# YuanxunLu/LiveSpeechPortraits

Measured on NVIDIA H100. Metric: 512x512 frames/sec (Feature2Face_G large / May.yaml), higher is better.
Workload: dtype fp16 hi+lo split operands (3 wgmma MMAs per K step), fp32 accumulate

## Files before the change

### livespeechportraits_b200/csrc/conv_wgmma.cuh

```cuda
#pragma once
#include <cuda_bf16.h>
#include <cuda_fp16.h>
#include "ptx.cuh"

namespace lspg {

constexpr int kTileM = 128;
constexpr int kChunk = 64;
constexpr int kATile = kTileM * 128;
constexpr int kMaxTaps = 9;
constexpr int kThreads = 384;
constexpr int kSmemBudget = 227 * 1024;

struct FastDiv {
  uint32_t mul, shr, d;
};
inline FastDiv make_fast_div(uint32_t d) {
  FastDiv f;
  f.d = d; f.mul = 0; f.shr = 0;
  if (d > 1) {
    uint32_t l = 0;
    while ((1u << l) < d) ++l;
    const uint64_t pw = 31 + l;
    f.mul = static_cast<uint32_t>(((1ull << pw) + d - 1) / d);
// ... 257 lines not shown
}

template <int CL>
__device__ __forceinline__ void release_stage(uint64_t* bar) {
  if constexpr (CL == 1) ptx::mbar_arrive(bar);
  else {
#pragma unroll
    for (int c = 0; c < CL; ++c) ptx::mbar_arrive_cluster(bar, static_cast<uint32_t>(c));
  }
}

template <int BN, int NL, bool TAIL>
__global__ void __launch_bounds__(kThreads, 1) conv_umma_kernel(const __grid_constant__ ConvParams p) {
  using Cfg = ConvCfg<BN, NL, TAIL>;
  const int t0 = static_cast<int>(blockIdx.x), tstep = static_cast<int>(gridDim.x);
  extern __shared__ uint8_t smem_raw[];
  uint8_t* smem = reinterpret_cast<uint8_t*>((reinterpret_cast<uintptr_t>(smem_raw) + 1023) & ~uintptr_t(1023));
  uint8_t* aux = smem + Cfg::kStages * Cfg::kStage;
  uint64_t* full_bar = reinterpret_cast<uint64_t*>(aux);
  uint64_t* empty_bar = full_bar + Cfg::kStages;
  float* tail_stg = reinterpret_cast<float*>(aux + kBarBytes);

  const int warp = __shfl_sync(0xffffffffu, static_cast<int>(threadIdx.x >> 5), 0);
  const int lane = threadIdx.x & 31;
  if (threadIdx.x == 0) { trace_stamp(p, 0); trace_time(p, false); }

  if (warp == 0 && lane == 0) {
    for (int i = 0; i < 4; ++i) ptx::prefetch_tmap(&p.a[i]);
    ptx::prefetch_tmap(&p.w);
    for (int i = 0; i < Cfg::kStages; ++i) {
      ptx::mbar_init(&full_bar[i], 1);
      ptx::mbar_init(&empty_bar[i], 2);
    }
    ptx::fence_mbar_init();
  }
  __syncthreads();
  ptx::pdl_launch_dependents();
  if (threadIdx.x == 0) trace_stamp(p, 1);

  int kb_per_tap = 0;
  for (int s = 0; s < p.n_src; ++s) kb_per_tap += p.chunks[s];
  const int num_kb = p.n_taps * kb_per_tap;

  if (warp == 0) {
    int pre = 0;
    if (t0 < p.total_tiles) {
      const TileCoord tc = decode_tile(p, t0);
      const int kb0 = tc.split * p.split_len;
      const int kb1 = (kb0 + p.split_len < num_kb) ? kb0 + p.split_len : num_kb;
      pre = (kb1 - kb0 < Cfg::kStages) ? kb1 - kb0 : Cfg::kStages;
      if (ptx::elect_one()) {
        for (int i = 0; i < pre; ++i) {
          uint8_t* st = smem + i * Cfg::kStage;
          ptx::mbar_expect_tx(&full_bar[i], Cfg::kStage);
#pragma unroll
          for (int l = 0; l < NL; ++l)
            ptx::tma_load_3d(&p.w, &full_bar[i], st + NL * kATile + l * Cfg::kBTile, (kb0 + i) * kChunk, tc.nt * BN,
                             l * p.n_phases + tc.z);
        }
      }
      __syncwarp();
    }
    ptx::pdl_wait();
    int stage = 0;
    uint32_t phase = 0;
    int issued = 0;
    int lt = 0;
    for (int t = t0; t < p.total_tiles; t += tstep, ++lt) {
      const TileCoord tc = decode_tile(p, t);
      const int kb0 = tc.split * p.split_len;
      const int kb1 = (kb0 + p.split_len < num_kb) ? kb0 + p.split_len : num_kb;
      if (lane == 0) trace_tile(p, lt, 6);
      for (int kb = kb0; kb < kb1; ++kb, ++issued) {
        const int tap = kb / kb_per_tap;
        const int rem = kb - tap * kb_per_tap;
        const int s = (rem < p.chunks[0]) ? 0 : 1;
        const int c = s ? rem - p.chunks[0] : rem;
        const int amap = p.tap_map[tc.z][tap];
        const int xx = tc.x0 + p.tap_dx[tc.z][tap];
        const int yy = tc.y0 + p.tap_dy[tc.z][tap];
        const bool early = issued < pre;
        if (!early) ptx::mbar_wait(&empty_bar[stage], phase ^ 1);
        if (ptx::elect_one()) {
          uint8_t* st = smem + stage * Cfg::kStage;
          if (!early) ptx::mbar_expect_tx(&full_bar[stage], Cfg::kStage);
#pragma unroll
          for (int l = 0; l < NL; ++l) {
            ptx::tma_load_5d(&p.a[amap + s], &full_bar[stage], st + l * kATile, c * kChunk, xx, yy, tc.n0, l);
            if (!early)
              ptx::tma_load_3d(&p.w, &full_bar[stage], st + NL * kATile + l * Cfg::kBTile, kb * kChunk, tc.nt * BN,
                               l * p.n_phases + tc.z);
          }
        }
        __syncwarp();
        if (++stage == Cfg::kStages) { stage = 0; phase ^= 1; }
      }
      if (lane == 0) trace_tile(p, lt, 7);
    }
  } else if (warp >= 4) {
    ptx::pdl_wait();
    const int cw = (warp >> 2) - 1;
    const bool wg_leader = (threadIdx.x & 127) == 0;
    int stage = 0;
    uint32_t phase = 0;
    int lt = 0;
    for (int t = t0; t < p.total_tiles; t += tstep, ++lt) {
      const TileCoord tc = decode_tile(p, t);
      const int kb0 = tc.split * p.split_len;
      const int kb1 = (kb0 + p.split_len < num_kb) ? kb0 + p.split_len : num_kb;
      if (threadIdx.x == 128) trace_tile(p, lt, 0);
      float acc[BN / 2];
#pragma unroll
      for (int i = 0; i < BN / 2; ++i) acc[i] = 0.0f;
      int prev = -1;
      for (int kb = kb0; kb < kb1; ++kb) {
        ptx::mbar_wait(&full_bar[stage], phase);
        if (threadIdx.x == 128 && kb == kb0) trace_tile(p, lt, 1);
        ptx::wgmma_fence();
        const uint32_t a0 = ptx::smem_u32(smem + stage * Cfg::kStage) + cw * 64 * 128;
        const uint32_t b0 = ptx::smem_u32(smem + stage * Cfg::kStage) + NL * kATile;
        const uint64_t a_hi = ptx::gmma_desc_sw128(a0);
        const uint64_t b_hi = ptx::gmma_desc_sw128(b0);
#pragma unroll
        for (int k = 0; k < kChunk / 16; ++k) {
          const uint32_t accum = (kb > kb0 || k > 0) ? 1u : 0u;
          ptx::wgmma_m64k16<BN, NL == 2>(acc, a_hi + 2 * k, b_hi + 2 * k, accum);
          if constexpr (NL == 2) {
            const uint64_t a_lo = ptx::gmma_desc_sw128(a0 + kATile);
            const uint64_t b_lo = ptx::gmma_desc_sw128(b0 + Cfg::kBTile);
            ptx::wgmma_m64k16<BN, true>(acc, a_hi + 2 * k, b_lo + 2 * k, 1u);
            ptx::wgmma_m64k16<BN, true>(acc, a_lo + 2 * k, b_hi + 2 * k, 1u);
          }
        }
        ptx::wgmma_commit();
        ptx::wgmma_wait<1>();
        if (prev >= 0 && wg_leader) release_stage<1>(&empty_bar[prev]);
        prev = stage;
        if (++stage == Cfg::kStages) { stage = 0; phase ^= 1; }
      }
      ptx::wgmma_wait<0>();
      if (prev >= 0 && wg_leader) release_stage<1>(&empty_bar[prev]);
      if (threadIdx.x == 128) trace_tile(p, lt, 2);
      epilogue_regs<BN, NL, TAIL>(p, acc, tc, t, 64 * cw, tail_stg + cw * 64 * kTailStride, 1 + cw);
      if (threadIdx.x == 128) trace_tile(p, lt, 3);
    }
  }
  if (threadIdx.x == 0) trace_time(p, true);
}


constexpr int kPatchSlot = 23 * 1024;
constexpr int kPatchStride = 23 * 1024;

constexpr int kProducerRegs = 40;
constexpr int kConsumerRegs = 232;
static_assert(128 * kProducerRegs + 256 * kConsumerRegs <= 65536, "register file of one SM");

template <int BN, int NL, bool TAIL>
struct PatchCfg {
  using Aux = AuxCfg<TAIL, 2 * kTileM>;
  static constexpr int kBTile = BN * 128;
  static constexpr int kTPS = TAIL ? 9 : (BN >= 128 ? (NL == 1 ? 2 : 1) : (NL == 1 ? 3 : 2));
  static constexpr int kAStage = NL * kPatchStride;
  static constexpr int kBStage = NL * kTPS * kBTile;
  static constexpr int kAStages = 2;
  static constexpr int kAvail = kSmemBudget - 1024 - Aux::kBytes - kAStages * kAStage;
  static constexpr int kBStagesRaw = kAvail / kBStage;
  static constexpr int kBStages = kBStagesRaw > 12 ? 12 : kBStagesRaw;
  static constexpr int kSmemBytes = 1024 + kAStages * kAStage + kBStages * kBStage + Aux::kBytes;
  static_assert(kBStages >= 2, "B ring needs at least two stages");
  static_assert(BN == 16 || BN == 64 || BN == 128, "instantiated N tiles");
};

template <int BN, int NL, bool TAIL, int CL>
__global__ void __launch_bounds__(kThreads, 1) conv_patch_kernel(const __grid_constant__ ConvParams p) {
  using Cfg = PatchCfg<BN, NL, TAIL>;
  const int t0 = static_cast<int>(blockIdx.x), tstep = static_cast<int>(gridDim.x);
  extern __shared__ uint8_t smem_raw[];
  uint8_t* smem = reinterpret_cast<uint8_t*>((reinterpret_cast<uintptr_t>(smem_raw) + 1023) & ~uintptr_t(1023));
  uint8_t* a_ring = smem;
  uint8_t* b_ring = a_ring + Cfg::kAStages * Cfg::kAStage;
  uint8_t* aux = b_ring + Cfg::kBStages * Cfg::kBStage;
  uint64_t* afull_bar = reinterpret_cast<uint64_t*>(aux);
  uint64_t* aempty_bar = afull_bar + Cfg::kAStages;
  uint64_t* bfull_bar = aempty_bar + Cfg::kAStages;
  uint64_t* bempty_bar = bfull_bar + Cfg::kBStages;
  uint64_t* turn_bar = bempty_bar + Cfg::kBStages;
  float* tail_stg = reinterpret_cast<float*>(aux + kBarBytes);

  const int warp = __shfl_sync(0xffffffffu, static_cast<int>(threadIdx.x >> 5), 0);
  const int lane = threadIdx.x & 31;
  if (threadIdx.x == 0) { trace_stamp(p, 0); trace_time(p, false); }

  if (warp == 0 && lane == 0) {
    for (int i = 0; i < 4; ++i) ptx::prefetch_tmap(&p.a[i]);
    ptx::prefetch_tmap(&p.w);
    for (int i = 0; i < Cfg::kAStages; ++i) { ptx::mbar_init(&afull_bar[i], 1); ptx::mbar_init(&aempty_bar[i], 1); }
    for (int i = 0; i < Cfg::kBStages; ++i) { ptx::mbar_init(&bfull_bar[i], 1); ptx::mbar_init(&bempty_bar[i], CL); }
    for (int i = 0; i < 2; ++i) ptx::mbar_init(&turn_bar[i], 1);
    ptx::fence_mbar_init();
  }
  __syncthreads();
  if (CL > 1) ptx::cluster_sync();
  const uint32_t crank = (CL > 1) ? ptx::cluster_ctarank() : 0u;
  constexpr uint16_t kMask = static_cast<uint16_t>((1u << CL) - 1u);
  ptx::pdl_launch_dependents();
  if (threadIdx.x == 0) trace_stamp(p, 1);

  int kb_per_tap = 0;
  for (int s = 0; s < p.n_src; ++s) kb_per_tap += p.chunks[s];
  const int patch_bytes = p.patch_w * p.patch_h * 128;
  const int n_groups = (p.n_taps + Cfg::kTPS - 1) / Cfg::kTPS;

  if (warp < 4) {
    ptx::setmaxnreg_dec<kProducerRegs>();
    if (warp == 0) {
      ptx::pdl_wait();
      int ia = 0, ib = 0;
      uint32_t pha = 0, phb = 0;
      int a_tile = t0, a_ci = -1;
      auto issue_a = [&]() {
        if (a_tile >= p.total_tiles) return;
        const TileCoord tc = decode_tile(p, a_tile);
        const int ci0 = tc.split * p.split_len;
        const int ci1 = (ci0 + p.split_len < kb_per_tap) ? ci0 + p.split_len : kb_per_tap;
        if (a_ci < 0) a_ci = ci0;
        const int s = (a_ci < p.chunks[0]) ? 0 : 1;
        const int c = (s == 0) ? a_ci : a_ci - p.chunks[0];
        ptx::mbar_wait(&aempty_bar[ia], pha ^ 1);
        if (ptx::elect_one()) {
          ptx::mbar_expect_tx(&afull_bar[ia], NL * patch_bytes);
#pragma unroll
          for (int l = 0; l < NL; ++l)
            ptx::tma_load_5d(&p.a[s], &afull_bar[ia], a_ring + ia * Cfg::kAStage + l * kPatchStride, c * kChunk,
                             tc.x0 + p.patch_dx0[tc.z], tc.y0 + p.patch_dy0[tc.z], tc.n0, l);
        }
        __syncwarp();
        if (++ia == Cfg::kAStages) { ia = 0; pha ^= 1; }
        if (++a_ci == ci1) { a_ci = -1; a_tile += tstep; }
      };
      issue_a();
      const int a_after_group = (n_groups > 1) ? 1 : 0;
      int lt = 0;
      for (int t = t0; t < p.total_tiles; t += tstep, ++lt) {
        const TileCoord tc = decode_tile(p, t);
        const int ci0 = tc.split * p.split_len;
        const int ci1 = (ci0 + p.split_len < kb_per_tap) ? ci0 + p.split_len : kb_per_tap;
        if (lane == 0) trace_tile(p, lt, 6);
        for (int ci = ci0; ci < ci1; ++ci) {
          for (int g = 0; g < n_groups; ++g) {
            ptx::mbar_wait(&bempty_bar[ib], phb ^ 1);
            if (ptx::elect_one()) {
              uint8_t* st = b_ring + ib * Cfg::kBStage;
              if constexpr (CL == 1 && NL == 1) {
                ptx::mbar_expect_tx(&bfull_bar[ib], Cfg::kBStage);
                ptx::tma_load_4d(&p.w, &bfull_bar[ib], st, ci * kChunk, tc.nt * BN, g * Cfg::kTPS, tc.z);
              } else {
                const int tap0 = g * Cfg::kTPS;
                const int ntap = (tap0 + Cfg::kTPS < p.n_taps) ? Cfg::kTPS : p.n_taps - tap0;
                ptx::mbar_expect_tx(&bfull_bar[ib], NL * ntap * Cfg::kBTile);
                constexpr int kRows = BN / CL;
                for (int ti = 0; ti < ntap; ++ti)
#pragma unroll
                  for (int l = 0; l < NL; ++l) {
                    uint8_t* dst = st + (ti * NL + l) * Cfg::kBTile + crank * kRows * 128;
                    if constexpr (CL == 1)
                      ptx::tma_load_4d(&p.w, &bfull_bar[ib], dst, ci * kChunk, tc.nt * BN, tap0 + ti, l * p.n_phases + tc.z);
                    else
                      ptx::tma_load_4d_mc(&p.w, &bfull_bar[ib], dst, ci * kChunk, tc.nt * BN + crank * kRows, tap0 + ti,
                                          l * p.n_phases + tc.z, kMask);
                  }
              }
            }
            __syncwarp();
            if (++ib == Cfg::kBStages) { ib = 0; phb ^= 1; }
            if (g == a_after_group) issue_a();
          }
        }
        if (lane == 0) trace_tile(p, lt, 7);
      }
    }
  } else {
    ptx::setmaxnreg_inc<kConsumerRegs>();
    ptx::pdl_wait();
    const int wg = (warp >> 2) - 1;
    const bool wg_leader = (threadIdx.x & 127) == 0;
    int ia = 0, ib = 0;
    uint32_t pha = 0, phb = 0;
    const uint32_t sbo = static_cast<uint32_t>(p.patch_w) * 128u;
    const uint32_t row_off = static_cast<uint32_t>(8 * p.patch_w) * 128u;
    const bool boff = p.desc_base_offset != 0;
    float* stg = tail_stg + wg * kTileM * kTailStride;
    int lt = 0;
    for (int t = t0; t < p.total_tiles; t += tstep, ++lt) {
      const TileCoord tc = decode_tile(p, t);
      const int ci0 = tc.split * p.split_len;
      const int ci1 = (ci0 + p.split_len < kb_per_tap) ? ci0 + p.split_len : kb_per_tap;
      if ((lt & 1) != wg) {
        ia += ci1 - ci0;
        pha ^= static_cast<uint32_t>(ia / Cfg::kAStages) & 1u;
        ia %= Cfg::kAStages;
        ib += (ci1 - ci0) * n_groups;
        phb ^= static_cast<uint32_t>(ib / Cfg::kBStages) & 1u;
        ib %= Cfg::kBStages;
        continue;
      }
      if (lt > 0) ptx::mbar_wait(&turn_bar[wg ^ 1], static_cast<uint32_t>((lt - 1) >> 1) & 1u);
      if (wg_leader) trace_tile(p, lt, 0);
      float acc[2][BN / 2];
#pragma unroll
      for (int h = 0; h < 2; ++h)
#pragma unroll
        for (int i = 0; i < BN / 2; ++i) acc[h][i] = 0.0f;
      int prev_b = -1, prev_a = -1;
      for (int ci = ci0; ci < ci1; ++ci) {
        ptx::mbar_wait(&afull_bar[ia], pha);
        const uint32_t a0 = ptx::smem_u32(a_ring + ia * Cfg::kAStage);
        for (int g = 0; g < n_groups; ++g) {
          ptx::mbar_wait(&bfull_bar[ib], phb);
          if (wg_leader && ci == ci0 && g == 0) trace_tile(p, lt, 1);
          ptx::wgmma_fence();
          const int tap0 = g * Cfg::kTPS;
          const uint32_t b0 = ptx::smem_u32(b_ring + ib * Cfg::kBStage);
#pragma unroll
          for (int i = 0; i < Cfg::kTPS; ++i) {
            const int tap = tap0 + i;
            if (i == 0 || tap < p.n_taps) {
              const uint32_t a_hi_addr = a0 + static_cast<uint32_t>(p.tap_row[tc.z][tap]) * 128u;
              const uint32_t b_hi_addr = b0 + static_cast<uint32_t>(i) * (NL * Cfg::kBTile);
              const uint64_t b_hi = ptx::gmma_desc_sw128(b_hi_addr);
              const uint64_t b_lo = ptx::gmma_desc_sw128(b_hi_addr + Cfg::kBTile);
#pragma unroll
              for (int k = 0; k < kChunk / 16; ++k) {
                const uint32_t accum = (ci > ci0 || tap > 0 || k > 0) ? 1u : 0u;
#pragma unroll
                for (int h = 0; h < 2; ++h) {
                  const uint64_t a_hi = ptx::gmma_desc_sw128(a_hi_addr + h * row_off, sbo, boff);
                  ptx::wgmma_m64k16<BN, NL == 2>(acc[h], a_hi + 2 * k, b_hi + 2 * k, accum);
                  if constexpr (NL == 2) {
                    const uint64_t a_lo = ptx::gmma_desc_sw128(a_hi_addr + h * row_off + kPatchStride, sbo, boff);
                    ptx::wgmma_m64k16<BN, true>(acc[h], a_hi + 2 * k, b_lo + 2 * k, 1u);
                    ptx::wgmma_m64k16<BN, true>(acc[h], a_lo + 2 * k, b_hi + 2 * k, 1u);
                  }
                }
              }
            }
          }
          ptx::wgmma_commit();
          if (ci == ci1 - 1 && g == n_groups - 1 && wg_leader) ptx::mbar_arrive(&turn_bar[wg]);
          ptx::wgmma_wait<1>();
          if (wg_leader) {
            if (prev_b >= 0) release_stage<CL>(&bempty_bar[prev_b]);
            if (prev_a >= 0) ptx::mbar_arrive(&aempty_bar[prev_a]);
          }
          prev_b = ib;
          prev_a = (g == n_groups - 1) ? ia : -1;
          if (++ib == Cfg::kBStages) { ib = 0; phb ^= 1; }
        }
        if (++ia == Cfg::kAStages) { ia = 0; pha ^= 1; }
      }
      ptx::wgmma_wait<0>();
      if (wg_leader) {
        if (prev_b >= 0) release_stage<CL>(&bempty_bar[prev_b]);
        if (prev_a >= 0) ptx::mbar_arrive(&aempty_bar[prev_a]);
      }
      if (wg_leader) trace_tile(p, lt, 2);
#pragma unroll
      for (int h = 0; h < 2; ++h)
        epilogue_regs<BN, NL, TAIL>(p, acc[h], tc, t, 64 * h, stg + 64 * h * kTailStride, 1 + wg);
      if (wg_leader) trace_tile(p, lt, 3);
    }
  }
  if (CL > 1) ptx::cluster_sync();
  if (threadIdx.x == 0) trace_time(p, true);
}

struct ReduceParams {
  const float* partial;
  const float* scale;
  const float* shift;
  const __nv_bfloat16* res;
  long long res_limb_stride;
  __nv_bfloat16* out;
  long long out_limb_stride;
  int32_t n_split, tiles_per_split, m_tiles, n_tiles, n_phases;
  int32_t tiles_x, tiles_y, tw_log2, th_log2, bn;
  int32_t batch, hs, ws, up, channels, relu, has_res, nl;
};

__global__ void __launch_bounds__(128) splitk_reduce_kernel(const ReduceParams p) {
  ptx::pdl_wait();
  ptx::pdl_launch_dependents();
  const int groups = p.bn >> 2;
  const long long total = static_cast<long long>(p.tiles_per_split) * kTileM * groups;
  for (long long e = blockIdx.x * static_cast<long long>(blockDim.x) + threadIdx.x; e < total;
       e += static_cast<long long>(gridDim.x) * blockDim.x) {
    const int g = static_cast<int>(e % groups);
    const long long r0 = e / groups;
    const int row = static_cast<int>(r0 % kTileM);
    const int tile = static_cast<int>(r0 / kTileM);
    const int mt = tile % p.m_tiles;
    const int r1 = tile / p.m_tiles;
    const int nt = r1 % p.n_tiles;
    const int z = r1 / p.n_tiles;
    const int tx = mt % p.tiles_x;
    const int r2 = mt / p.tiles_x;
    const int ty = r2 % p.tiles_y;
    const int tn = r2 / p.tiles_y;
    const int tw = row & ((1 << p.tw_log2) - 1);
    const int th = (row >> p.tw_log2) & ((1 << p.th_log2) - 1);
    const int nb = row >> (p.tw_log2 + p.th_log2);
    const int n = (tn << (7 - p.tw_log2 - p.th_log2)) + nb;
    const int y = (ty << p.th_log2) + th, x = (tx << p.tw_log2) + tw;
    if (n >= p.batch || y >= p.hs || x >= p.ws) continue;
    float acc[4] = {0.f, 0.f, 0.f, 0.f};
    const size_t split_stride = static_cast<size_t>(p.tiles_per_split) * kTileM * p.bn;
    const float* src0 = p.partial + (static_cast<size_t>(tile) * kTileM + row) * p.bn + g * 4;
    int s = 0;
    for (; s + 16 <= p.n_split; s += 16) {
      float4 v[16];
#pragma unroll
      for (int u = 0; u < 16; ++u) v[u] = *reinterpret_cast<const float4*>(src0 + (s + u) * split_stride);
#pragma unroll
      for (int u = 0; u < 16; ++u) {
        acc[0] += v[u].x; acc[1] += v[u].y; acc[2] += v[u].z; acc[3] += v[u].w;
      }
    }
    for (; s + 4 <= p.n_split; s += 4) {
      float4 v[4];
#pragma unroll
      for (int u = 0; u < 4; ++u) v[u] = *reinterpret_cast<const float4*>(src0 + (s + u) * split_stride);
#pragma unroll
      for (int u = 0; u < 4; ++u) { acc[0] += v[u].x; acc[1] += v[u].y; acc[2] += v[u].z; acc[3] += v[u].w; }
    }
    for (; s < p.n_split; ++s) {
      const float4 a = *reinterpret_cast<const float4*>(src0 + s * split_stride);
      acc[0] += a.x; acc[1] += a.y; acc[2] += a.z; acc[3] += a.w;
    }
    const int ch = nt * p.bn + g * 4;
    const int oh = p.up ? 2 * p.hs : p.hs, ow = p.up ? 2 * p.ws : p.ws;
    const int oy = p.up ? 2 * y + (z >> 1) : y, ox = p.up ? 2 * x + (z & 1) : x;
    const size_t off = ((static_cast<size_t>(n) * oh + oy) * ow + ox) * p.channels + ch;
    const float4 sc = *reinterpret_cast<const float4*>(p.scale + ch), sh = *reinterpret_cast<const float4*>(p.shift + ch);
    float yv[4] = {fmaf(acc[0], sc.x, sh.x), fmaf(acc[1], sc.y, sh.y), fmaf(acc[2], sc.z, sh.z), fmaf(acc[3], sc.w, sh.w)};
    if (p.has_res) {
      for (int l = 0; l < p.nl; ++l) {
        const uint2 r = *reinterpret_cast<const uint2*>(p.res + l * p.res_limb_stride + off);
        if (p.nl == 2) {
          yv[0] += unpack_lo<true>(r.x); yv[1] += unpack_hi<true>(r.x); yv[2] += unpack_lo<true>(r.y); yv[3] += unpack_hi<true>(r.y);
        } else {
          yv[0] += bf16_lo(r.x); yv[1] += bf16_hi(r.x); yv[2] += bf16_lo(r.y); yv[3] += bf16_hi(r.y);
        }
      }
    }
    if (p.relu) {
#pragma unroll
      for (int i = 0; i < 4; ++i) yv[i] = fmaxf(yv[i], 0.f);
    }
    if (p.nl == 2) {
      uint2 o, lo;
      o.x = pack2<true>(yv[0], yv[1]); o.y = pack2<true>(yv[2], yv[3]);
      lo.x = pack2<true>(yv[0] - unpack_lo<true>(o.x), yv[1] - unpack_hi<true>(o.x));
      lo.y = pack2<true>(yv[2] - unpack_lo<true>(o.y), yv[3] - unpack_hi<true>(o.y));
      *reinterpret_cast<uint2*>(p.out + off) = o;
      *reinterpret_cast<uint2*>(p.out + p.out_limb_stride + off) = lo;
    } else {
      uint2 o;
      o.x = pack_bf16x2(yv[0], yv[1]); o.y = pack_bf16x2(yv[2], yv[3]);
      *reinterpret_cast<uint2*>(p.out + off) = o;
    }
  }
}

}
```

### livespeechportraits_b200/csrc/lspg.cu

```cuda
#include <cuda.h>
#include <cuda_runtime.h>

#include <algorithm>
#include <cmath>
#include <cstdarg>
#include <cstdio>
#include <cstdlib>
#include <cstring>
#include <functional>
#include <map>
#include <memory>
#include <string>
#include <tuple>
#include <utility>
#include <vector>

#include "../../include/lspg.h"
#include "aux_kernels.cuh"
#include "raster.cuh"
#include "conv_wgmma.cuh"

namespace {

using namespace lspg;
// ... 592 lines not shown
    p.n_tiles = L.cout_pad / pl.bn;
    p.n_phases = L.n_phases;
    p.tiles_per_split = g.tiles_per_split;
    p.fd_tps = make_fast_div(g.tiles_per_split);
    p.fd_m_tiles = make_fast_div(p.tiles_x * p.tiles_y * p.tiles_n);
    p.fd_n_tiles = make_fast_div(p.n_tiles);
    p.fd_tiles_x = make_fast_div(p.tiles_x);
    p.fd_tiles_y = make_fast_div(p.tiles_y);
    p.n_split = g.n_split; p.split_len = g.split_len;
    p.total_tiles = g.tiles_per_split * g.n_split;
    p.partial = reinterpret_cast<float*>(ws_scratch);
    pl.split = g.n_split > 1;
    p.n_taps = L.n_taps; p.n_src = L.n_src;
    p.chunks[0] = L.cin[0] / 64; p.chunks[1] = L.n_src == 2 ? L.cin[1] / 64 : 0;
    p.relu = L.relu; p.has_res = L.res >= 0 ? 1 : 0;
    p.batch = B; p.hs = Hs; p.ws = Ws;
    const bool f16 = NL > 1;
    p.scale = f16 ? L.d_scale_par : L.d_scale; p.shift = L.d_shift; p.out_f32 = nullptr;
    memcpy(p.tap_map, L.tap_map, sizeof(p.tap_map));
    memcpy(p.tap_dx, L.tap_dx, sizeof(p.tap_dx));
    memcpy(p.tap_dy, L.tap_dy, sizeof(p.tap_dy));
    int rc;
    for (int s = 0; s < L.n_src; ++s) {
      const TensorInfo& t = h->tensors[L.src[s]];
      const int Ht = H >> t.shift, Wt = W >> t.shift;
      void* tb = ws + P->tensor_off[L.src[s]];
      const size_t ls = P->tensor_limb_stride[L.src[s]];
      if (L.kind == K_S2) {
        for (int q = 0; q < 4; ++q)
          if ((rc = make_act_map(h, &p.a[q], tb, ls, NL, t.channels, B, Ht, Wt, true, q >> 1, q & 1, tw, th, nb))) return rc;
      } else {
        if ((rc = make_act_map(h, &p.a[s], tb, ls, NL, t.channels, B, Ht, Wt, false, 0, 0, abox_w, abox_h, abox_n))) return rc;
      }
    }
    const int used = (L.kind == K_S2) ? 4 : L.n_src;
    for (int q = used; q < 4; ++q) p.a[q] = p.a[0];
    if (pl.patch) {
      static const bool no_cluster = getenv("LSPG_NO_CLUSTER") != nullptr;
      pl.cluster = ((!no_cluster && g.n_split == 1 && g.m_tiles % 2 == 0 && g.tiles_per_split >= h->num_sms)) ? 2 : 1;
      if (pl.cluster == 1 && NL == 1) rc = make_weight_map_taps(h, &p.w, L, pl.bn, patch_tps(pl.bn, NL, L.kind == K_TAIL), NL);
      else rc = make_weight_map_taps(h, &p.w, L, pl.bn / pl.cluster, 1, NL);
      if (rc) return rc;
    } else {
      if ((rc = make_weight_map(h, &p.w, L, pl.bn, NL))) return rc;
    }
    if (L.kind != K_TAIL) {
      const TensorInfo& t = h->tensors[L.out];
      void* tb = ws + P->tensor_off[L.out];
      const size_t ls = P->tensor_limb_stride[L.out];
      p.out_ptr = reinterpret_cast<__nv_bfloat16*>(tb);
      p.out_limb_stride = static_cast<long long>(ls / 2);
      p.out_channels = t.channels;
      p.out_up = (L.kind == K_UP) ? 1 : 0;
      if (L.res >= 0) {
        const TensorInfo& r = h->tensors[L.res];
        p.res_ptr = reinterpret_cast<const __nv_bfloat16*>(ws + P->tensor_off[L.res]);
        p.res_limb_stride = static_cast<long long>(P->tensor_limb_stride[L.res] / 2);
        p.res_channels = r.channels;
      }
    }
    pl.grid = p.total_tiles < h->num_sms ? p.total_tiles : h->num_sms;
    if (pl.cluster > 1) pl.grid -= pl.grid % pl.cluster;
    {
      const char* tl = getenv("LSPG_TRACE_LAYER");
      if (tl && atoi(tl) == static_cast<int>(P->layers.size())) {
        if (!h->trace_buf) CUDA_TRY(cudaMalloc(&h->trace_buf, sizeof(unsigned long long) * 256 * kTraceSlots));
        CUDA_TRY(cudaMemset(h->trace_buf, 0, sizeof(unsigned long long) * 256 * kTraceSlots));
        p.trace = h->trace_buf;
        const char* ts = getenv("LSPG_TRACE_SKIP");
        p.trace_skip = ts ? atoi(ts) : 0;
      }
    }
    if (pl.split) {
      ReduceParams& r = pl.red;
      memset(&r, 0, sizeof(r));
      r.partial = p.partial; r.scale = p.scale; r.shift = L.d_shift;
      r.out = reinterpret_cast<__nv_bfloat16*>(ws + P->tensor_off[L.out]);
      r.out_limb_stride = static_cast<long long>(P->tensor_limb_stride[L.out] / 2);
      if (L.res >= 0) {
        r.res = reinterpret_cast<const __nv_bfloat16*>(ws + P->tensor_off[L.res]);
        r.res_limb_stride = static_cast<long long>(P->tensor_limb_stride[L.res] / 2);
      }
      r.n_split = g.n_split; r.tiles_per_split = g.tiles_per_split; r.m_tiles = g.m_tiles; r.n_tiles = g.n_tiles;
      r.n_phases = L.n_phases; r.tiles_x = p.tiles_x; r.tiles_y = p.tiles_y; r.tw_log2 = p.tw_log2; r.th_log2 = p.th_log2;
      r.bn = g.bn; r.batch = B; r.hs = Hs; r.ws = Ws; r.up = (L.kind == K_UP) ? 1 : 0; r.channels = L.cout_pad;
      r.relu = L.relu; r.has_res = L.res >= 0 ? 1 : 0; r.nl = NL;
      const long long work = static_cast<long long>(g.tiles_per_split) * kTileM * (g.bn / 4);
      pl.red_blocks = static_cast<int>(std::min<long long>((work + 127) / 128, 8LL * h->num_sms));
    }
    P->layers.push_back(pl);
  }
  return LSPG_OK;
}

template <typename... KArgs, typename... Args>
cudaError_t launch_pdl_cluster(void (*kernel)(KArgs...), dim3 grid, dim3 block, size_t smem, cudaStream_t st, int cluster,
                               Args&&... args) {
  static const bool no_pdl = getenv("LSPG_NO_PDL") != nullptr;
  cudaLaunchConfig_t cfg{};
  cfg.gridDim = grid; cfg.blockDim = block; cfg.dynamicSmemBytes = smem; cfg.stream = st;
  cudaLaunchAttribute attr[2];
  int n = 0;
  if (!no_pdl) {
    attr[n].id = cudaLaunchAttributeProgrammaticStreamSerialization;
    attr[n].val.programmaticStreamSerializationAllowed = 1;
    ++n;
  }
  if (cluster > 1) {
    attr[n].id = cudaLaunchAttributeClusterDimension;
    attr[n].val.clusterDim.x = static_cast<unsigned>(cluster);
    attr[n].val.clusterDim.y = 1;
    attr[n].val.clusterDim.z = 1;
    ++n;
  }
  cfg.attrs = attr; cfg.numAttrs = n;
  return cudaLaunchKernelEx(&cfg, kernel, std::forward<Args>(args)...);
}

template <typename... KArgs, typename... Args>
cudaError_t launch_pdl(void (*kernel)(KArgs...), dim3 grid, dim3 block, size_t smem, cudaStream_t st, Args&&... args) {
  return launch_pdl_cluster(kernel, grid, block, smem, st, 1, std::forward<Args>(args)...);
}

template <typename K>
int ensure_smem(K kernel, int bytes, int device, unsigned long long* done_mask) {
  const unsigned long long bit = 1ull << (device & 63);
  if (!(*done_mask & bit)) {
    CUDA_TRY(cudaFuncSetAttribute(kernel, cudaFuncAttributeMaxDynamicSharedMemorySize, bytes));
    *done_mask |= bit;
  }
  return LSPG_OK;
}

const void* g_last_func = nullptr;

template <int BN, int NL, bool TAIL>
int launch_conv(const ConvParams& p, int grid, int device, cudaStream_t st) {
  using Cfg = ConvCfg<BN, NL, TAIL>;
  static unsigned long long done = 0;
  int rc = ensure_smem(conv_umma_kernel<BN, NL, TAIL>, Cfg::kSmemBytes, device, &done);
  if (rc) return rc;
  g_last_func = reinterpret_cast<const void*>(conv_umma_kernel<BN, NL, TAIL>);
  CUDA_TRY(launch_pdl_cluster(conv_umma_kernel<BN, NL, TAIL>, dim3(grid), dim3(kThreads), Cfg::kSmemBytes, st, 1, p));
  return LSPG_OK;
}

template <int BN, int NL, bool TAIL, int CL>
int launch_patch(const ConvParams& p, int grid, int device, cudaStream_t st) {
  using Cfg = PatchCfg<BN, NL, TAIL>;
  static unsigned long long done = 0;
  int rc = ensure_smem(conv_patch_kernel<BN, NL, TAIL, CL>, Cfg::kSmemBytes, device, &done);
  if (rc) return rc;
  g_last_func = reinterpret_cast<const void*>(conv_patch_kernel<BN, NL, TAIL, CL>);
  CUDA_TRY(launch_pdl_cluster(conv_patch_kernel<BN, NL, TAIL, CL>, dim3(grid), dim3(kThreads), Cfg::kSmemBytes, st, CL, p));
  return LSPG_OK;
}

template <int BN, int NL, bool TAIL>
int launch_patch_cl(const ConvParams& p, int grid, int cluster, int device, cudaStream_t st) {
  return cluster == 2 ? launch_patch<BN, NL, TAIL, 2>(p, grid, device, st) : launch_patch<BN, NL, TAIL, 1>(p, grid, device, st);
}

int launch_layer(const PlanLayer& pl, int kind, int NL, int device, cudaStream_t st) {
  if (pl.patch) {
    const int c = pl.cluster;
    if (kind == K_TAIL) return NL == 1 ? launch_patch_cl<16, 1, true>(pl.prm, pl.grid, c, device, st) : launch_patch_cl<16, 2, true>(pl.prm, pl.grid, c, device, st);
    if (pl.bn == 128) return NL == 1 ? launch_patch_cl<128, 1, false>(pl.prm, pl.grid, c, device, st) : launch_patch_cl<128, 2, false>(pl.prm, pl.grid, c, device, st);
    return NL == 1 ? launch_patch_cl<64, 1, false>(pl.prm, pl.grid, c, device, st) : launch_patch_cl<64, 2, false>(pl.prm, pl.grid, c, device, st);
  }
  if (kind == K_TAIL) return NL == 1 ? launch_conv<16, 1, true>(pl.prm, pl.grid, device, st) : launch_conv<16, 2, true>(pl.prm, pl.grid, device, st);
  if (pl.bn == 128) return NL == 1 ? launch_conv<128, 1, false>(pl.prm, pl.grid, device, st) : launch_conv<128, 2, false>(pl.prm, pl.grid, device, st);
  return NL == 1 ? launch_conv<64, 1, false>(pl.prm, pl.grid, device, st) : launch_conv<64, 2, false>(pl.prm, pl.grid, device, st);
}

struct PackArgs {
  const float* fm; long long fs; const float* cand; long long cs; int in_nc;
  __nv_bfloat16* dst; long long limb_stride; int batch, height, width;
  int blocks;
};

PackArgs make_pack_args(const lspg_ctx* h, const Plan* P, const IoKey& io) {
  PackArgs a;
  a.fm = io.fm; a.fs = io.fm_bstride; a.cand = io.cand; a.cs = io.cand_bstride; a.in_nc = h->in_nc;
  a.dst = reinterpret_cast<__nv_bfloat16*>(static_cast<uint8_t*>(P->workspace) + P->tensor_off[0]);
  a.limb_stride = static_cast<long long>(P->tensor_limb_stride[0] / 2);
  a.batch = P->batch; a.height = P->height; a.width = P->width;
  const long long total = static_cast<long long>(P->batch) * (P->height / 2) * (P->width / 2);
  a.blocks = static_cast<int>((total + 127) / 128);
  if (a.blocks > h->num_sms * 16) a.blocks = h->num_sms * 16;
  return a;
}

void set_tail_io(ConvParams* prm, const IoKey& io) {
  prm->out_f32 = io.u8 ? nullptr : static_cast<float*>(io.out);
  prm->out_u8 = io.u8 ? static_cast<uint8_t*>(io.out) : nullptr;
}

int enqueue_forward(lspg_ctx* h, Plan* P, const IoKey& io, cudaStream_t st, bool debug_sync, bool profile) {
  const int NL = nl_of(P->mode);
  int rc;
  std::vector<cudaEvent_t>* evs = nullptr;
  if (profile && h->prof_used < 256) {
    if (h->prof_used == h->prof_events.size()) {
      std::vector<cudaEvent_t> set(h->layers.size() + 2);
      for (auto& e : set) CUDA_TRY(cudaEventCreate(&e));
      h->prof_events.push_back(set);
    }
    evs = &h->prof_events[h->prof_used++];
    CUDA_TRY(cudaEventRecord((*evs)[0], st));
  }
  {
    const PackArgs a = make_pack_args(h, P, io);
    if (NL == 1)
      CUDA_TRY(launch_pdl(pack_input_s2d_kernel<1>, dim3(a.blocks), dim3(128), 0, st, a.fm, a.fs, a.cand, a.cs, a.in_nc, a.dst, a.limb_stride, a.batch, a.height, a.width));
    else
      CUDA_TRY(launch_pdl(pack_input_s2d_kernel<2>, dim3(a.blocks), dim3(128), 0, st, a.fm, a.fs, a.cand, a.cs, a.in_nc, a.dst, a.limb_stride, a.batch, a.height, a.width));
    if (debug_sync) CUDA_TRY(cudaStreamSynchronize(st));
    if (evs) CUDA_TRY(cudaEventRecord((*evs)[1], st));
  }
  for (size_t i = 0; i < h->layers.size(); ++i) {
    PlanLayer& pl = P->layers[i];
    if (h->layers[i].kind == K_TAIL) set_tail_io(&pl.prm, io);
    if ((rc = launch_layer(pl, h->layers[i].kind, NL, h->device, st))) return rc;
    if (h->layers[i].kind == K_TAIL) h->tail_func = g_last_func;
    if (pl.split) {
      CUDA_TRY(launch_pdl(splitk_reduce_kernel, dim3(pl.red_blocks), dim3(128), 0, st, pl.red));
    }
    if (evs) CUDA_TRY(cudaEventRecord((*evs)[i + 2], st));
    if (debug_sync) {
      cudaError_t e = cudaStreamSynchronize(st);
      if (e != cudaSuccess)
        return fail(LSPG_ECUDA, "layer %zu (kind %d, %s, bn %d, grid %d, tiles %d) failed: %s", i, h->layers[i].kind,
                    h->layers[i].conv_key.c_str(), pl.bn, pl.grid, pl.prm.total_tiles, cudaGetErrorString(e));
    }
  }
  return LSPG_OK;
}

void free_plan_graph(Plan* P) {
  if (P->exec) cudaGraphExecDestroy(P->exec);
  if (P->graph) cudaGraphDestroy(P->graph);
  P->exec = nullptr; P->graph = nullptr; P->pack_node = P->tail_node = nullptr;
}

int capture_plan_graph(lspg_ctx* h, Plan* P, const IoKey& io) {
  const int NL = nl_of(P->mode);
  if (!h->capture_stream) CUDA_TRY(cudaStreamCreateWithFlags(&h->capture_stream, cudaStreamNonBlocking));
  cudaGraph_t graph = nullptr;
  CUDA_TRY(cudaStreamBeginCapture(h->capture_stream, cudaStreamCaptureModeThreadLocal));
  int rc = enqueue_forward(h, P, io, h->capture_stream, false, false);
  cudaError_t ce = cudaStreamEndCapture(h->capture_stream, &graph);
  if (rc) { if (graph) cudaGraphDestroy(graph); return rc; }
  if (ce != cudaSuccess) return fail(LSPG_ECUDA, "cudaStreamEndCapture failed: %s", cudaGetErrorString(ce));
  cudaGraphExec_t exec = nullptr;
  ce = cudaGraphInstantiate(&exec, graph, 0);
  if (ce != cudaSuccess) { cudaGraphDestroy(graph); return fail(LSPG_ECUDA, "cudaGraphInstantiate failed: %s", cudaGetErrorString(ce)); }
  P->graph = graph; P->exec = exec; P->io = io;
  P->pack_node = P->tail_node = nullptr;
  const void* pack_func = NL == 1 ? reinterpret_cast<const void*>(pack_input_s2d_kernel<1>)
                                  : reinterpret_cast<const void*>(pack_input_s2d_kernel<2>);
  size_t n = 0;
  if (cudaGraphGetNodes(graph, nullptr, &n) == cudaSuccess && n > 0) {
    std::vector<cudaGraphNode_t> nodes(n);
    if (cudaGraphGetNodes(graph, nodes.data(), &n) == cudaSuccess) {
      for (size_t i = 0; i < n; ++i) {
        cudaGraphNodeType ty;
        if (cudaGraphNodeGetType(nodes[i], &ty) != cudaSuccess || ty != cudaGraphNodeTypeKernel) continue;
        cudaKernelNodeParams np{};
        if (cudaGraphKernelNodeGetParams(nodes[i], &np) != cudaSuccess) continue;
        if (np.func == pack_func) { P->pack_node = nodes[i]; P->pack_np = np; }
        else if (np.func == h->tail_func) { P->tail_node = nodes[i]; P->tail_np = np; }
      }
    }
  }
  cudaGetLastError();
  ++h->n_captures;
  return LSPG_OK;
}

int update_graph_io(lspg_ctx* h, Plan* P, const IoKey& io) {
  if (!P->pack_node || !P->tail_node) return fail(LSPG_ECUDA, "graph nodes of the packer / tail conv were not identified");
  PackArgs a = make_pack_args(h, P, io);
  void* pargs[10] = {&a.fm, &a.fs, &a.cand, &a.cs, &a.in_nc, &a.dst, &a.limb_stride, &a.batch, &a.height, &a.width};
  cudaKernelNodeParams np = P->pack_np;
  np.kernelParams = pargs; np.extra = nullptr;
  CUDA_TRY(cudaGraphExecKernelNodeSetParams(P->exec, P->pack_node, &np));
  ConvParams prm = P->layers.back().prm;
  set_tail_io(&prm, io);
  void* targs[1] = {&prm};
  np = P->tail_np;
  np.kernelParams = targs; np.extra = nullptr;
  CUDA_TRY(cudaGraphExecKernelNodeSetParams(P->exec, P->tail_node, &np));
  P->layers.back().prm = prm;
  P->io = io;
  ++h->n_io_updates;
  return LSPG_OK;
}

}

extern "C" {

const char* lspg_last_error(void) { return g_err.c_str(); }

int lspg_create(lspg_handle* out, int variant, int ngf, int num_downs, int in_nc, int out_nc, int device) {
  if (!out) return fail(LSPG_EINVAL, "out is NULL");
  *out = nullptr;
// ... 380 lines not shown
```

Before: 725.5.

## Split each patch-kernel consumer team across two warpgroups for BN=64 tiles

For BN=64 non-tail patch convolutions, each ping-pong consumer team becomes two warpgroups instead of one, and each warpgroup computes one 64-row half of the 128-row tile. The block grows to 640 threads, with per-role register limits and barrier arrival counts scaled to match. The aim is more warps issuing wgmma and running the epilogue in parallel, which hides latency for the narrow-N tiles. The cost is fewer registers per consumer and more barrier arrivals per stage.

```diff
diff --git a/livespeechportraits_b200/csrc/conv_wgmma.cuh b/livespeechportraits_b200/csrc/conv_wgmma.cuh
--- a/livespeechportraits_b200/csrc/conv_wgmma.cuh
+++ b/livespeechportraits_b200/csrc/conv_wgmma.cuh
@@ -433,12 +433,14 @@
 constexpr int kPatchSlot = 23 * 1024;
 constexpr int kPatchStride = 23 * 1024;
 
-constexpr int kProducerRegs = 40;
-constexpr int kConsumerRegs = 232;
-static_assert(128 * kProducerRegs + 256 * kConsumerRegs <= 65536, "register file of one SM");
-
 template <int BN, int NL, bool TAIL>
 struct PatchCfg {
+  static constexpr int kWPT = (BN == 64 && !TAIL) ? 2 : 1;
+  static constexpr int kThreads = 128 * (1 + 2 * kWPT);
+  static constexpr int kLaunchRegs = 65536 / kThreads / 8 * 8;
+  static constexpr int kProducerRegs = kWPT == 1 ? 40 : 32;
+  static constexpr int kConsumerRegs = kWPT == 1 ? 232 : 112;
+  static_assert(128 * kProducerRegs + 256 * kWPT * kConsumerRegs <= kThreads * kLaunchRegs, "CTA register allocation");
   using Aux = AuxCfg<TAIL, 2 * kTileM>;
   static constexpr int kBTile = BN * 128;
   static constexpr int kTPS = TAIL ? 9 : (BN >= 128 ? (NL == 1 ? 2 : 1) : (NL == 1 ? 3 : 2));
@@ -454,8 +456,9 @@
 };
 
 template <int BN, int NL, bool TAIL, int CL>
-__global__ void __launch_bounds__(kThreads, 1) conv_patch_kernel(const __grid_constant__ ConvParams p) {
+__global__ void __launch_bounds__(PatchCfg<BN, NL, TAIL>::kThreads, 1) conv_patch_kernel(const __grid_constant__ ConvParams p) {
   using Cfg = PatchCfg<BN, NL, TAIL>;
+  constexpr int kWPT = Cfg::kWPT;
   const int t0 = static_cast<int>(blockIdx.x), tstep = static_cast<int>(gridDim.x);
   extern __shared__ uint8_t smem_raw[];
   uint8_t* smem = reinterpret_cast<uint8_t*>((reinterpret_cast<uintptr_t>(smem_raw) + 1023) & ~uintptr_t(1023));
@@ -476,9 +479,9 @@
   if (warp == 0 && lane == 0) {
     for (int i = 0; i < 4; ++i) ptx::prefetch_tmap(&p.a[i]);
     ptx::prefetch_tmap(&p.w);
-    for (int i = 0; i < Cfg::kAStages; ++i) { ptx::mbar_init(&afull_bar[i], 1); ptx::mbar_init(&aempty_bar[i], 1); }
-    for (int i = 0; i < Cfg::kBStages; ++i) { ptx::mbar_init(&bfull_bar[i], 1); ptx::mbar_init(&bempty_bar[i], CL); }
-    for (int i = 0; i < 2; ++i) ptx::mbar_init(&turn_bar[i], 1);
+    for (int i = 0; i < Cfg::kAStages; ++i) { ptx::mbar_init(&afull_bar[i], 1); ptx::mbar_init(&aempty_bar[i], kWPT); }
+    for (int i = 0; i < Cfg::kBStages; ++i) { ptx::mbar_init(&bfull_bar[i], 1); ptx::mbar_init(&bempty_bar[i], kWPT * CL); }
+    for (int i = 0; i < 2; ++i) ptx::mbar_init(&turn_bar[i], kWPT);
     ptx::fence_mbar_init();
   }
   __syncthreads();
@@ -494,7 +497,7 @@
   const int n_groups = (p.n_taps + Cfg::kTPS - 1) / Cfg::kTPS;
 
   if (warp < 4) {
-    ptx::setmaxnreg_dec<kProducerRegs>();
+    ptx::setmaxnreg_dec<Cfg::kProducerRegs>();
     if (warp == 0) {
       ptx::pdl_wait();
       int ia = 0, ib = 0;
@@ -562,22 +565,26 @@
       }
     }
   } else {
-    ptx::setmaxnreg_inc<kConsumerRegs>();
+    ptx::setmaxnreg_inc<Cfg::kConsumerRegs>();
     ptx::pdl_wait();
-    const int wg = (warp >> 2) - 1;
+    constexpr int kHalves = 2 / kWPT;
+    const int cw = (warp >> 2) - 1;
+    const int team = cw / kWPT, member = cw % kWPT;
     const bool wg_leader = (threadIdx.x & 127) == 0;
+    const bool lead = wg_leader && member == 0;
     int ia = 0, ib = 0;
     uint32_t pha = 0, phb = 0;
     const uint32_t sbo = static_cast<uint32_t>(p.patch_w) * 128u;
     const uint32_t row_off = static_cast<uint32_t>(8 * p.patch_w) * 128u;
+    const uint32_t a_member = static_cast<uint32_t>(member * kHalves) * row_off;
     const bool boff = p.desc_base_offset != 0;
-    float* stg = tail_stg + wg * kTileM * kTailStride;
+    float* stg = tail_stg + team * kTileM * kTailStride;
     int lt = 0;
     for (int t = t0; t < p.total_tiles; t += tstep, ++lt) {
       const TileCoord tc = decode_tile(p, t);
       const int ci0 = tc.split * p.split_len;
       const int ci1 = (ci0 + p.split_len < kb_per_tap) ? ci0 + p.split_len : kb_per_tap;
-      if ((lt & 1) != wg) {
+      if ((lt & 1) != team) {
         ia += ci1 - ci0;
         pha ^= static_cast<uint32_t>(ia / Cfg::kAStages) & 1u;
         ia %= Cfg::kAStages;
@@ -586,20 +593,20 @@
         ib %= Cfg::kBStages;
         continue;
       }
-      if (lt > 0) ptx::mbar_wait(&turn_bar[wg ^ 1], static_cast<uint32_t>((lt - 1) >> 1) & 1u);
-      if (wg_leader) trace_tile(p, lt, 0);
-      float acc[2][BN / 2];
-#pragma unroll
-      for (int h = 0; h < 2; ++h)
+      if (lt > 0) ptx::mbar_wait(&turn_bar[team ^ 1], static_cast<uint32_t>((lt - 1) >> 1) & 1u);
+      if (lead) trace_tile(p, lt, 0);
+      float acc[kHalves][BN / 2];
+#pragma unroll
+      for (int h = 0; h < kHalves; ++h)
 #pragma unroll
         for (int i = 0; i < BN / 2; ++i) acc[h][i] = 0.0f;
       int prev_b = -1, prev_a = -1;
       for (int ci = ci0; ci < ci1; ++ci) {
         ptx::mbar_wait(&afull_bar[ia], pha);
-        const uint32_t a0 = ptx::smem_u32(a_ring + ia * Cfg::kAStage);
+        const uint32_t a0 = ptx::smem_u32(a_ring + ia * Cfg::kAStage) + a_member;
         for (int g = 0; g < n_groups; ++g) {
           ptx::mbar_wait(&bfull_bar[ib], phb);
-          if (wg_leader && ci == ci0 && g == 0) trace_tile(p, lt, 1);
+          if (lead && ci == ci0 && g == 0) trace_tile(p, lt, 1);
           ptx::wgmma_fence();
           const int tap0 = g * Cfg::kTPS;
           const uint32_t b0 = ptx::smem_u32(b_ring + ib * Cfg::kBStage);
@@ -615,7 +622,7 @@
               for (int k = 0; k < kChunk / 16; ++k) {
                 const uint32_t accum = (ci > ci0 || tap > 0 || k > 0) ? 1u : 0u;
 #pragma unroll
-                for (int h = 0; h < 2; ++h) {
+                for (int h = 0; h < kHalves; ++h) {
                   const uint64_t a_hi = ptx::gmma_desc_sw128(a_hi_addr + h * row_off, sbo, boff);
                   ptx::wgmma_m64k16<BN, NL == 2>(acc[h], a_hi + 2 * k, b_hi + 2 * k, accum);
                   if constexpr (NL == 2) {
@@ -628,7 +635,7 @@
             }
           }
           ptx::wgmma_commit();
-          if (ci == ci1 - 1 && g == n_groups - 1 && wg_leader) ptx::mbar_arrive(&turn_bar[wg]);
+          if (ci == ci1 - 1 && g == n_groups - 1 && wg_leader) ptx::mbar_arrive(&turn_bar[team]);
           ptx::wgmma_wait<1>();
           if (wg_leader) {
             if (prev_b >= 0) release_stage<CL>(&bempty_bar[prev_b]);
@@ -645,11 +652,13 @@
         if (prev_b >= 0) release_stage<CL>(&bempty_bar[prev_b]);
         if (prev_a >= 0) ptx::mbar_arrive(&aempty_bar[prev_a]);
       }
-      if (wg_leader) trace_tile(p, lt, 2);
-#pragma unroll
-      for (int h = 0; h < 2; ++h)
-        epilogue_regs<BN, NL, TAIL>(p, acc[h], tc, t, 64 * h, stg + 64 * h * kTailStride, 1 + wg);
-      if (wg_leader) trace_tile(p, lt, 3);
+      if (lead) trace_tile(p, lt, 2);
+#pragma unroll
+      for (int h = 0; h < kHalves; ++h) {
+        const int rh = member * kHalves + h;
+        epilogue_regs<BN, NL, TAIL>(p, acc[h], tc, t, 64 * rh, stg + 64 * rh * kTailStride, 1 + team);
+      }
+      if (lead) trace_tile(p, lt, 3);
     }
   }
   if (CL > 1) ptx::cluster_sync();
diff --git a/livespeechportraits_b200/csrc/lspg.cu b/livespeechportraits_b200/csrc/lspg.cu
--- a/livespeechportraits_b200/csrc/lspg.cu
+++ b/livespeechportraits_b200/csrc/lspg.cu
@@ -768,7 +768,7 @@
   int rc = ensure_smem(conv_patch_kernel<BN, NL, TAIL, CL>, Cfg::kSmemBytes, device, &done);
   if (rc) return rc;
   g_last_func = reinterpret_cast<const void*>(conv_patch_kernel<BN, NL, TAIL, CL>);
-  CUDA_TRY(launch_pdl_cluster(conv_patch_kernel<BN, NL, TAIL, CL>, dim3(grid), dim3(kThreads), Cfg::kSmemBytes, st, CL, p));
+  CUDA_TRY(launch_pdl_cluster(conv_patch_kernel<BN, NL, TAIL, CL>, dim3(grid), dim3(Cfg::kThreads), Cfg::kSmemBytes, st, CL, p));
   return LSPG_OK;
 }
 
```

Result: no change. 721.8 (median of 6 runs) (-0.5%).
